# Bendabir/torch-kafka

Hardware: AMD Instinct MI355X
Metric: Kafka records/sec to GPU with per-batch commit, at 1/2/4/8 MI355X (higher is better)
Workload: dtype bf16

## Files before the change

torchkafka_amd/csrc/hip/json_span.hip:

```cpp
#include <hip/hip_runtime.h>

#include <stdexcept>
#include <string>

#include "dtypes.h"
#include "json_scan_dev.h"
#include "span_decode.h"
#include "span_device.h"

namespace tkh {

namespace {

using span::kBlock;
using span::kFront;
using span::kThreads;
using span::kWinBytes;
constexpr int kBufs = 2;
constexpr int kWaves = kThreads / 64;
constexpr int kMaxRows = int(tk::kJsonSpanMaxSegRows);
constexpr int kRowsPerThread = kMaxRows / kThreads;

__device__ __forceinline__ uint32_t align16(uint32_t x) { return (x + 15u) & ~15u; }

__global__ __launch_bounds__(kBlock) void json_stage_kernel(JsonStageLaunch a) {
  __shared__ __attribute__((aligned(16))) uint8_t bufs[kBufs][kWinBytes];
  __shared__ int32_t rel[kMaxRows];
  __shared__ int32_t tln[kMaxRows];
  __shared__ uint32_t dst[kMaxRows];
  __shared__ __attribute__((aligned(256))) uint32_t tab[span::kNibLdsWords];
  __shared__ span::RowWins rw;
  __shared__ uint32_t wcrc[kWaves];
  __shared__ uint32_t wsum[kWaves];
  __shared__ int32_t bad;

  const int t = int(threadIdx.x), lane = t & 63, wv = t >> 6;
  const int P = a.parts;
  const SpanDevSeg& sg = a.s[int(blockIdx.x) / P];
  const JsonStageBatch& bo = a.b[sg.batch];
  const uint32_t row_begin = sg.row_begin;
  const int32_t nrows = int32_t(sg.row_end - row_begin);
  const uint32_t flags = sg.flags;
  const int32_t trunc = bo.trunc_len;

  if (flags & tk::kSegHostRows) {
    if (wv != 0 || int(blockIdx.x) % P != 0) return;
    uint32_t off = sg.stage_off;
    for (int32_t rr = 0; rr < nrows; ++rr) {
      const int64_t row = int64_t(row_begin) + rr;
      const tk::JsonSpanRow d = bo.rows[row];
      if (d.tlen >= 0) continue;
      const int32_t n_out = trunc >= 0 && d.count > trunc ? trunc : d.count;
      const float* __restrict__ src = reinterpret_cast<const float*>(bo.slot + d.pos);
      float* __restrict__ o = reinterpret_cast<float*>(bo.stage + off);
      for (int32_t k = lane; k < n_out; k += 64) o[k] = src[k];
      if (lane == 0) {
        bo.desc[row] = JsonRowDesc{off, -1, d.count, n_out};
        if (bo.ctr) atomicMax(bo.ctr, (static_cast<unsigned long long>(bo.ctr_tag) << 32) | uint32_t(max(n_out, 0)));
      }
      off += align16(uint32_t(n_out) * 4u);
    }
    return;
  }

  const uint32_t len = sg.len;
  const int32_t head = int32_t(reinterpret_cast<uintptr_t>(sg.src) & 15u);
  const bool do_crc = (flags & tk::kSegCrc) != 0;
  const int32_t lo_b = kFront + head, hi_b = lo_b + int32_t(len);
  const span::Windows W(lo_b, hi_b);
  const span::Part pt = span::part_of(P, W.nw);

  const uint32_t crc = span::pipeline<kBufs>(
      sg.src, W, pt.k0, pt.k1, bufs, tab, a.tabs, lo_b + ((flags & tk::kSegCrcFirst) ? 21 : 0), do_crc,
      (flags & tk::kSegCrcFirst) != 0,
      [&] {
        const int64_t base = int64_t(sg.log_pos) - int64_t(head) - kFront;
        for (int32_t r = t; r < nrows; r += kThreads) {
          const tk::JsonSpanRow d = bo.rows[row_begin + uint32_t(r)];
          const int32_t r0 = d.tlen >= 0 ? int32_t(int64_t(d.pos) - base) : 0;
          rel[r] = r0;
          tln[r] = d.tlen < 0 ? -1 : (r0 < lo_b || r0 + d.tlen > hi_b) ? -2 : d.tlen;
        }
        span::row_wins_init(rw, W.nw);
        if (t == 0) bad = 0;
      },
      [&] {
        const bool cw = t < kThreads;
        uint32_t sz[kRowsPerThread], local = 0;
#pragma unroll
        for (int i = 0; i < kRowsPerThread; ++i) {
          const int32_t r = t * kRowsPerThread + i;
          sz[i] = cw && r < nrows && tln[r] >= 0 ? align16(uint32_t(tln[r])) : 0u;
          local += sz[i];
        }
        uint32_t incl = local;
#pragma unroll
        for (int o = 1; o < 64; o <<= 1) {
          const uint32_t u = __shfl_up(incl, o, 64);
          if (lane >= o) incl += u;
        }
        if (cw && lane == 63) wsum[wv] = incl;
        __syncthreads();
        if (!cw) return;
        uint32_t off = sg.stage_off + incl - local;
        for (int w = 0; w < wv; ++w) off += wsum[w];
#pragma unroll
        for (int i = 0; i < kRowsPerThread; ++i) {
          const int32_t r = t * kRowsPerThread + i;
          if (r < nrows) {
            dst[r] = off;
            const int32_t T = tln[r];
            if (pt.q != 0) {
            } else if (T == -2) {
              bo.desc[row_begin + uint32_t(r)] = JsonRowDesc{off, 0, 0, 0};
              bad = 1;
            } else if (T >= 0) {
              const int32_t c = bo.rows[row_begin + uint32_t(r)].count;
              const int32_t n_out = c < 0 ? 0 : trunc >= 0 && c > trunc ? trunc : c;
              bo.desc[row_begin + uint32_t(r)] = JsonRowDesc{off, T, c, n_out};
            }
          }
          off += sz[i];
        }
        for (int32_t r0w = 0; r0w < nrows; r0w += kThreads) {
          const int32_t r = r0w + t;
          const int32_t T = r < nrows ? tln[r] : -1;
          const int32_t r0 = r < nrows ? rel[r] : 0;
          span::row_wins_add(rw, W.nw, r0w + (t & ~63), T > 0, W.win_of(r0), W.win_of(r0 + ((T - 1) & ~15)));
        }
      },
      [&](int k, const uint8_t* buf, int32_t off) {
        const int32_t ra = rw.lo[k], rb = rw.hi[k];
        if (ra >= rb) return;
        const int32_t own_lo = W.own_lo(k), own_hi = W.own_hi(k);
        span::for_rows(
            ra, rb, false,
            [&](int32_t rr, int32_t* ulo, int32_t* uhi) {
              const int32_t T = tln[rr], r0 = rel[rr];
              *ulo = span::unit_from(r0, own_lo);
              *uhi = min(T > 0 ? (T + 15) >> 4 : 0, span::unit_from(r0, own_hi));
            },
            [&](int32_t rr, int32_t u) {
              *reinterpret_cast<uint4*>(bo.stage + dst[rr] + 16u * uint32_t(u)) =
                  span::lds16_row(reinterpret_cast<const uint4*>(buf), rel[rr] + 16 * u + off);
            });
      });

  if (do_crc) {
    if (t < kThreads) span::crc_merge(crc, wcrc);
    __syncthreads();
    if (t == 0)
      span::crc_finish(wcrc, flags, sg.crc, sg.seg, bo.err, bo.partials, P, pt.q,
                       a.part_acc + 2 * pt.seg);
  }
  if (t == 0 && bad) span::report_bad_segment(bo.err, sg.seg);
}

__global__ __launch_bounds__(256) void json_count_kernel(JsonGroupArgs a) {
  const int lane = int(threadIdx.x) & 63;
  const int64_t g = int64_t(blockIdx.x) * 4 + int64_t(threadIdx.x >> 6);
  if (g >= a.row_base[a.n]) return;
  int bk = 0;
#pragma unroll
  for (int k = 1; k < kMaxGroup; ++k) bk += (k < a.n && g >= a.row_base[k]) ? 1 : 0;
  if (!a.ctr[bk]) return;
  const int64_t r = g - a.row_base[bk];
  JsonRowDesc* desc = const_cast<JsonRowDesc*>(a.rows[bk]) + r;
  const JsonRowDesc d = *desc;
  if (d.count != tk::kJsonCountOnDevice || d.tlen < 0) return;
  const int32_t T = d.tlen;
  if (uint64_t(d.off) + ((uint64_t(T) + 15u) & ~uint64_t(15)) > a.vals_cap[bk]) return;
  const uint8_t* __restrict__ text = a.vals[bk] + d.off;
  int32_t guess = 0;
  const int32_t count = json_scan_row([&](int32_t c) { return *reinterpret_cast<const uint4*>(text + c); },
                                      [&](int32_t i) { return uint32_t(text[i]); }, T, lane, &guess);
  if (lane == 0) {
    const bool host = count < 0;
    const int32_t c = host ? guess : count;
    const int32_t trunc = a.trunc[bk];
    const int32_t n_out = trunc >= 0 && c > trunc ? trunc : c;
    *desc = JsonRowDesc{d.off, host ? tk::kJsonCountOnDevice : T, c, n_out};
    const unsigned long long tag = static_cast<unsigned long long>(a.ctr_tag[bk]) << 32;
    atomicMax(const_cast<unsigned long long*>(a.ctr[bk]), tag | uint32_t(max(n_out, 0)));
    if (host) atomicMax(const_cast<unsigned long long*>(a.ctr[bk]) + 1, tag | 1u);
  }
}

}

void launch_json_count(const JsonGroupArgs& a, hipStream_t stream) {
  if (a.n < 1 || a.n > kMaxGroup) throw std::invalid_argument("json count: group size out of range");
  const int64_t total = a.row_base[a.n];
  if (total <= 0) return;
  if (total > INT32_MAX) throw std::invalid_argument("json count: too many rows");
  for (int k = 0; k < a.n; ++k) {
    if (a.ctr[k] && (reinterpret_cast<uintptr_t>(a.vals[k]) % 16 || reinterpret_cast<uintptr_t>(a.rows[k]) % 16 ||
                     a.row_base[k + 1] < a.row_base[k]))
      throw std::invalid_argument("json count: malformed group");
  }
  hipLaunchKernelGGL(json_count_kernel, dim3(unsigned((total + 3) / 4)), dim3(256), 0, stream, a);
  hipError_t e = hipGetLastError();
  if (e != hipSuccess) throw std::runtime_error(std::string("json count launch: ") + hipGetErrorString(e));
}

void launch_json_stage(const JsonStageLaunch& a0, hipStream_t stream) {
  JsonStageLaunch a = a0;
  a.parts = check_parts(a.parts, a.part_acc, "json stage");
  if (a.n_seg < 0 || a.n_seg > kMaxLaunchSegs) throw std::invalid_argument("json stage: bad segment count");
  if (a.n_seg == 0) return;
  for (int i = 0; i < a.n_seg; ++i) {
    const SpanDevSeg& s = a.s[i];
    const bool host = (s.flags & tk::kSegHostRows) != 0;
    if ((!host && (s.len == 0 || s.len > tk::kSpanSegMax || s.src == nullptr)) || s.row_end < s.row_begin ||
        s.row_end - s.row_begin > tk::kJsonSpanMaxSegRows || s.batch >= kMaxGroup || a.b[s.batch].stage == nullptr ||
        a.b[s.batch].desc == nullptr || (s.stage_off & 15u) != 0)
      throw std::invalid_argument("json stage: malformed segment");
  }
  hipLaunchKernelGGL(json_stage_kernel, dim3(unsigned(a.n_seg * a.parts)), dim3(kBlock), 0, stream, a);
  hipError_t e = hipGetLastError();
  if (e != hipSuccess) throw std::runtime_error(std::string("json stage launch: ") + hipGetErrorString(e));
}

void prewarm_json_span_kernels() {
  hipFuncAttributes attr;
  (void)hipFuncGetAttributes(&attr, reinterpret_cast<const void*>(&json_stage_kernel));
  (void)hipFuncGetAttributes(&attr, reinterpret_cast<const void*>(&json_count_kernel));
}

}
```

torchkafka_amd/csrc/hip/span_decode.hip:

```cpp
#include <hip/hip_runtime.h>

#include <algorithm>
#include <stdexcept>
#include <string>

#include "convert.h"
#include "span_decode.h"
#include "span_device.h"

namespace tkh {

namespace {

using span::kBlock;
using span::kFront;
using span::kThreads;
using span::kWinBytes;
constexpr int kBufs = 3;

template <typename S>
__device__ __forceinline__ S lds_elem(const uint32_t* b32, int32_t b) {
  const int32_t w = b >> 2, sh = b & 3;
  if constexpr (sizeof(S) <= 4) {
    const uint32_t x = __builtin_amdgcn_alignbyte(b32[w + 1], b32[w], sh);
    S v;
    __builtin_memcpy(&v, &x, sizeof(S));
    return v;
  } else {
    const uint32_t x0 = b32[w], x1 = b32[w + 1], x2 = b32[w + 2];
    const uint32_t o[2] = {__builtin_amdgcn_alignbyte(x1, x0, sh), __builtin_amdgcn_alignbyte(x2, x1, sh)};
    S v;
    __builtin_memcpy(&v, o, sizeof(S));
    return v;
  }
}

template <typename S, typename D, bool AFFINE>
__global__ __launch_bounds__(kBlock) void span_decode_kernel(SpanLaunch a, const float* __restrict__ shift,
                                                               const float* __restrict__ scale) {
  using C = Conv<S, D, IsIntDst<D>::value>;
  constexpr int kPer = 16 / int(sizeof(S));
  __shared__ __attribute__((aligned(16))) uint8_t bufs[kBufs][kWinBytes];
  __shared__ int32_t rel[tk::kSpanMaxSegRows];
  __shared__ __attribute__((aligned(256))) uint32_t tab[span::kNibLdsWords];
  __shared__ span::RowWins rw;
  __shared__ uint32_t wcrc[kThreads / 64];

  const int t = int(threadIdx.x);
  const int P = a.parts;
  const SpanDevSeg& sg = a.s[int(blockIdx.x) / P];
  const SpanBatchOut& bo = a.b[sg.batch];
  const uint32_t len = sg.len, flags = sg.flags;
  const int32_t head = int32_t(reinterpret_cast<uintptr_t>(sg.src) & 15u);
  const uint32_t row_begin = sg.row_begin;
  const int32_t nrows = int32_t(sg.row_end - row_begin);
  const bool do_crc = (flags & tk::kSegCrc) != 0;
  const int32_t lo_b = kFront + head, hi_b = lo_b + int32_t(len);
  const span::Windows W(lo_b, hi_b);
  const span::Part pt = span::part_of(P, W.nw);
  const int64_t RE = a.row_elems;
  const int32_t G = int32_t((RE + kPer - 1) / kPer);
  const int32_t row_bytes = int32_t(RE * int64_t(sizeof(S)));
  D* __restrict__ out = static_cast<D*>(bo.out);

  auto group = [&](const uint8_t* buf, int32_t off, int32_t own_lo, int32_t own_hi, int32_t rr, int32_t gi,
                   bool row_wave) {
    const uint32_t* b32 = reinterpret_cast<const uint32_t*>(buf);
    const int32_t e0 = gi * kPer;
    const int32_t b0 = rel[rr] + e0 * int32_t(sizeof(S));
    const int64_t rem = RE - e0;
    const int nel = rem < kPer ? int(rem) : kPer;
    if (b0 + nel * int32_t(sizeof(S)) <= lo_b || b0 >= hi_b) return;
    const int32_t key = b0 > lo_b ? b0 : lo_b;
    if (key < own_lo || key >= own_hi) return;
    D* __restrict__ orow = out + int64_t(row_begin + uint32_t(rr)) * RE;
    if (nel == kPer && b0 >= lo_b && b0 + 16 <= hi_b) {
      const uint4 o = row_wave ? span::lds16_row(reinterpret_cast<const uint4*>(buf), b0 + off)
                               : span::lds16(reinterpret_cast<const uint4*>(buf), b0 + off);
      S sv[kPer];
      __builtin_memcpy(sv, &o, 16);
      Vec<D, kPer> ov;
#pragma unroll
      for (int k = 0; k < kPer; ++k) {
        if constexpr (AFFINE)
          ov.v[k] = C::apply(sv[k], shift[e0 + k], scale[e0 + k], true);
        else
          ov.v[k] = C::apply(sv[k], 0.f, 1.f, false);
      }
      if (a.vec_store) {
        *reinterpret_cast<Vec<D, kPer>*>(orow + e0) = ov;
      } else {
#pragma unroll
        for (int k = 0; k < kPer; ++k) orow[e0 + k] = ov.v[k];
      }
    } else {
      for (int k = 0; k < nel; ++k) {
        const int32_t be = b0 + k * int32_t(sizeof(S));
        if (be < lo_b || be + int32_t(sizeof(S)) > hi_b) continue;
        const S sv = lds_elem<S>(b32, be + off);
        if constexpr (AFFINE)
          orow[e0 + k] = C::apply(sv, shift[e0 + k], scale[e0 + k], true);
        else
          orow[e0 + k] = C::apply(sv, 0.f, 1.f, false);
      }
    }
  };

  const uint32_t crc = span::pipeline<kBufs>(
      sg.src, W, pt.k0, pt.k1, bufs, tab, a.tabs, lo_b + ((flags & tk::kSegCrcFirst) ? 21 : 0), do_crc,
      (flags & tk::kSegCrcFirst) != 0,
      [&] {
        const int64_t base = int64_t(sg.log_pos) - int64_t(head) - kFront;
        for (int32_t r = t; r < nrows; r += kThreads) rel[r] = int32_t(int64_t(bo.row_pos[row_begin + uint32_t(r)]) - base);
        span::row_wins_init(rw, W.nw);
      },
      [&] {
        if (t >= kThreads) return;
        for (int32_t r0w = 0; r0w < nrows; r0w += kThreads) {
          const int32_t r = r0w + t;
          const int32_t r0 = r < nrows ? rel[r] : 0;
          const bool in = r < nrows && r0 + row_bytes > lo_b && r0 < hi_b;
          const int32_t kf = r0 > lo_b ? r0 : lo_b, kl = min(r0 + (G - 1) * 16, hi_b - 1);
          span::row_wins_add(rw, W.nw, r0w + (t & ~63), in, W.win_of(kf), W.win_of(kl));
        }
        if (sg.seg == 0 && pt.q == 0 && bo.ext_words)
          for (uint32_t i = uint32_t(t); i < bo.ext_words; i += kThreads) bo.ext_out[i] = bo.ext_src[i];
      },
      [&](int k, const uint8_t* buf, int32_t off) {
        const int32_t ra = rw.lo[k], rb = rw.hi[k];
        if (ra >= rb) return;
        const int32_t own_lo = W.own_lo(k), own_hi = W.own_hi(k);
        if (G >= 32) {
          span::for_rows(
              ra, rb, G > 128,
              [&](int32_t rr, int32_t* ulo, int32_t* uhi) {
                const int32_t r0 = rel[rr];
                *ulo = k == 0 ? (r0 >= lo_b ? 0 : (lo_b - r0) >> 4) : span::unit_from(r0, own_lo);
                *uhi = min(G, span::unit_from(r0, own_hi));
              },
              [&](int32_t rr, int32_t gi) { group(buf, off, own_lo, own_hi, rr, gi, true); });
        } else {
          const int32_t total = (rb - ra) * G;
          for (int32_t p = t; p < total; p += kThreads) {
            const int32_t q = p / G;
            group(buf, off, own_lo, own_hi, ra + q, p - q * G, false);
          }
        }
      });

  if (do_crc) {
    if (t < kThreads) span::crc_merge(crc, wcrc);
    __syncthreads();
    if (t == 0)
      span::crc_finish(wcrc, flags, sg.crc, sg.seg, bo.err, bo.partials, P, pt.q,
                       a.part_acc + 2 * pt.seg);
  }
}

template <typename S, typename D>
__global__ __launch_bounds__(kBlock) void varlen_span_kernel(VarSpanLaunch a, D pad) {
  using C = Conv<S, D, IsIntDst<D>::value>;
  constexpr int kWaves = kThreads / 64;
  constexpr int kPer = 16 / int(sizeof(S));
  __shared__ __attribute__((aligned(16))) uint8_t bufs[kBufs][kWinBytes];
  __shared__ int32_t rel[tk::kJsonSpanMaxSegRows];
  __shared__ int32_t nout[tk::kJsonSpanMaxSegRows];
  __shared__ __attribute__((aligned(256))) uint32_t tab[span::kNibLdsWords];
  __shared__ span::RowWins rw;
  __shared__ uint32_t wcrc[kWaves];
  __shared__ int32_t bad;

  const int t = int(threadIdx.x), lane = t & 63, wv = t >> 6;
  const int P = a.parts;
  const SpanDevSeg& sg = a.s[int(blockIdx.x) / P];
  const VarSpanBatch& bo = a.b[sg.batch];
  const uint32_t row_begin = sg.row_begin;
  const int32_t nrows = int32_t(sg.row_end - row_begin);
  const uint32_t flags = sg.flags;
  const int64_t L = bo.L;
  const int32_t trunc = bo.trunc_len;
  D* __restrict__ out = static_cast<D*>(bo.out);
  auto finish = [&](D* orow, int64_t row, int64_t n_out) {
    for (int64_t k = n_out + lane; k < L; k += 64) orow[k] = pad;
    if (bo.mask) {
      uint8_t* mrow = bo.mask + row * L;
      for (int64_t k = lane; k < L; k += 64) mrow[k] = uint8_t(k < n_out);
    }
    if (bo.lengths && lane == 0) bo.lengths[row] = n_out;
  };

  if (flags & tk::kSegHostRows) {
    if (wv >= kWaves || int(blockIdx.x) % P != 0) return;
    for (int32_t rr = wv; rr < nrows; rr += kWaves) {
      const int64_t row = int64_t(row_begin) + rr;
      const tk::JsonSpanRow d = bo.rows[row];
      if (d.tlen >= 0) continue;
      int64_t n_out = trunc >= 0 && d.count > trunc ? trunc : d.count;
      n_out = n_out < L ? n_out : L;
      const S* __restrict__ v = reinterpret_cast<const S*>(bo.slot + d.pos);
      D* orow = out + row * L;
      for (int64_t k = lane; k < n_out; k += 64) orow[k] = C::apply(v[k], 0.f, 1.f, false);
      finish(orow, row, n_out);
    }
    return;
  }

  const uint32_t len = sg.len;
  const int32_t head = int32_t(reinterpret_cast<uintptr_t>(sg.src) & 15u);
  const bool do_crc = (flags & tk::kSegCrc) != 0;
  const int32_t lo_b = kFront + head, hi_b = lo_b + int32_t(len);
  const span::Windows W(lo_b, hi_b);
  const span::Part pt = span::part_of(P, W.nw);

  const uint32_t crc = span::pipeline<kBufs>(
      sg.src, W, pt.k0, pt.k1, bufs, tab, a.tabs, lo_b + ((flags & tk::kSegCrcFirst) ? 21 : 0), do_crc,
      (flags & tk::kSegCrcFirst) != 0,
      [&] {
        const int64_t base = int64_t(sg.log_pos) - int64_t(head) - kFront;
        for (int32_t r = t; r < nrows; r += kThreads) {
          const tk::JsonSpanRow d = bo.rows[row_begin + uint32_t(r)];
          rel[r] = d.tlen >= 0 ? int32_t(int64_t(d.pos) - base) : 0;
          int32_t n = -1;
          if (d.tlen >= 0) {
            int64_t n_out = trunc >= 0 && d.count > trunc ? trunc : d.count;
            n_out = n_out < L ? n_out : L;
            const bool ok = rel[r] >= lo_b && rel[r] + d.tlen <= hi_b && int64_t(d.count) * int64_t(sizeof(S)) == d.tlen;
            n = ok ? int32_t(n_out) : -2;
          }
          nout[r] = n;
        }
        span::row_wins_init(rw, W.nw);
        if (t == 0) bad = 0;
      },
      [&] {
        if (t >= kThreads) return;
        for (int32_t rr = wv; rr < nrows; rr += kWaves) {
          const int32_t n = nout[rr];
          if (n == -1) continue;
          if (n == -2 && lane == 0) bad = 1;
          const int64_t row = int64_t(row_begin) + rr;
          if (pt.q == 0) finish(out + row * L, row, n < 0 ? 0 : n);
        }
        for (int32_t r0w = 0; r0w < nrows; r0w += kThreads) {
          const int32_t r = r0w + t;
          const int32_t n = r < nrows ? nout[r] : 0;
          const int32_t r0 = r < nrows ? rel[r] : 0;
          const int32_t units = n > 0 ? (n + kPer - 1) / kPer : 0;
          span::row_wins_add(rw, W.nw, r0w + (t & ~63), units > 0, W.win_of(r0), W.win_of(r0 + 16 * (units - 1)));
        }
      },
      [&](int k, const uint8_t* buf, int32_t off) {
        const int32_t ra = rw.lo[k], rb = rw.hi[k];
        if (ra >= rb) return;
        const int32_t own_lo = W.own_lo(k), own_hi = W.own_hi(k);
        const uint32_t* b32 = reinterpret_cast<const uint32_t*>(buf);
        span::for_rows(
            ra, rb, false,
            [&](int32_t rr, int32_t* ulo, int32_t* uhi) {
              const int32_t n = nout[rr], r0 = rel[rr];
              const int32_t units = n > 0 ? (n + kPer - 1) / kPer : 0;
              *ulo = span::unit_from(r0, own_lo);
              *uhi = min(units, span::unit_from(r0, own_hi));
            },
            [&](int32_t rr, int32_t u) {
              const int32_t n = nout[rr], r0 = rel[rr];
              D* orow = out + (int64_t(row_begin) + rr) * L;
              const int32_t e0 = u * kPer, b0 = r0 + 16 * u + off;
              if (bo.reserved && e0 + kPer <= n) {
                const uint4 o = span::lds16_row(reinterpret_cast<const uint4*>(buf), b0);
                S sv[kPer];
                __builtin_memcpy(sv, &o, 16);
                Vec<D, kPer> ov;
#pragma unroll
                for (int q = 0; q < kPer; ++q) ov.v[q] = C::apply(sv[q], 0.f, 1.f, false);
                *reinterpret_cast<Vec<D, kPer>*>(orow + e0) = ov;
              } else {
                for (int q = 0; q < kPer && e0 + q < n; ++q)
                  orow[e0 + q] = C::apply(lds_elem<S>(b32, b0 + q * int32_t(sizeof(S))), 0.f, 1.f, false);
              }
            });
      });

  if (do_crc) {
    if (t < kThreads) span::crc_merge(crc, wcrc);
    __syncthreads();
    if (t == 0)
      span::crc_finish(wcrc, flags, sg.crc, sg.seg, bo.err, bo.partials, P, pt.q,
                       a.part_acc + 2 * pt.seg);
  }
  if (t == 0 && bad) span::report_bad_segment(bo.err, sg.seg);
}

template <typename S, typename D>
void launch_var_span_t(const VarSpanLaunch& a, double pad, hipStream_t stream) {
  D padv;
  if constexpr (IsIntDst<D>::value) padv = D(int64_t(pad)); else padv = Store<D>::cvt(float(pad));
  hipLaunchKernelGGL((varlen_span_kernel<S, D>), dim3(unsigned(a.n_seg * a.parts)), dim3(kBlock), 0, stream, a, padv);
}

template <typename S, typename D>
void launch_span_t(const SpanLaunch& a, const float* shift, const float* scale, hipStream_t stream) {
  if (a.n_seg <= 0) return;
  const dim3 grid(unsigned(a.n_seg * a.parts));
  if (shift)
    hipLaunchKernelGGL((span_decode_kernel<S, D, true>), grid, dim3(kBlock), 0, stream, a, shift, scale);
  else
    hipLaunchKernelGGL((span_decode_kernel<S, D, false>), grid, dim3(kBlock), 0, stream, a, shift, scale);
}

}

int check_parts(int parts, const uint32_t* acc, const char* what) {
  if (parts <= 1) return 1;
  if ((parts != 2 && parts != 4 && parts != tk::kSpanMaxParts) || acc == nullptr)
    throw std::invalid_argument(std::string(what) + ": parts must be 1, 2, 4 or 8 (with accumulator words)");
  return parts;
}

void prewarm_span_kernels(int device) {
  (void)device;
  hipFuncAttributes attr;
  (void)hipFuncGetAttributes(&attr, reinterpret_cast<const void*>(&span_decode_kernel<float, __bf16, false>));
  (void)hipFuncGetAttributes(&attr, reinterpret_cast<const void*>(&span_decode_kernel<float, float, false>));
  (void)hipFuncGetAttributes(&attr, reinterpret_cast<const void*>(&span_decode_kernel<float, _Float16, false>));
  (void)hipFuncGetAttributes(&attr, reinterpret_cast<const void*>(&span_decode_kernel<float, fp8e4m3, false>));
}

void check_var_span(const VarSpanLaunch& a, int src_dt, int dst_dt) {
  check_parts(a.parts, a.part_acc, "var span");
  if (a.n_seg < 0 || a.n_seg > kMaxLaunchSegs) throw std::invalid_argument("var span: bad segment count");
  if (!is_float_dt(dst_dt) && is_float_dt(src_dt))
    throw std::invalid_argument("collate: float records cannot be cast to an integer dtype");
  for (int i = 0; i < a.n_seg; ++i) {
    const SpanDevSeg& s = a.s[i];
    const bool host = (s.flags & tk::kSegHostRows) != 0;
    if ((!host && (s.len == 0 || s.len > tk::kSpanSegMax || s.src == nullptr)) || s.row_end < s.row_begin ||
        s.row_end - s.row_begin > tk::kJsonSpanMaxSegRows || s.batch >= kMaxGroup ||
        (a.b[s.batch].L > 0 && a.b[s.batch].out == nullptr))
      throw std::invalid_argument("var span: malformed segment");
    const VarSpanBatch& b = a.b[s.batch];
    if (b.err == nullptr || (s.row_end > s.row_begin && (b.rows == nullptr || (host && b.slot == nullptr))) ||
        (!host && (s.flags & tk::kSegCrc) && (a.tabs == nullptr || b.partials == nullptr)))
      throw std::invalid_argument("var span: a segment without its status word, row table, slot or CRC tables");
  }
}

void launch_var_span(const VarSpanLaunch& a0, int src_dt, int dst_dt, double pad, hipStream_t stream) {
  check_var_span(a0, src_dt, dst_dt);
  VarSpanLaunch a = a0;
  a.parts = check_parts(a.parts, a.part_acc, "var span");
  if (a.n_seg == 0) return;
  TK_DISPATCH_SRC(launch_var_span_t, a, pad, stream)
  hipError_t e = hipGetLastError();
  if (e != hipSuccess) throw std::runtime_error(std::string("var span launch: ") + hipGetErrorString(e));
}

void check_span_decode(const SpanLaunch& a, int src_dt, int dst_dt, const float* shift, const float* scale) {
  check_parts(a.parts, a.part_acc, "span decode");
  if (a.n_seg < 0 || a.n_seg > kMaxLaunchSegs) throw std::invalid_argument("span decode: bad segment count");
  if (!is_float_dt(dst_dt) && is_float_dt(src_dt))
    throw std::invalid_argument("collate: float records cannot be cast to an integer dtype");
  if (shift && !is_float_dt(dst_dt)) throw std::invalid_argument("collate: normalisation needs a float dtype");
  if ((shift == nullptr) != (scale == nullptr)) throw std::invalid_argument("span decode: shift and scale go together");
  if (a.n_seg > 0 && a.row_elems < 1) throw std::invalid_argument("span decode: row_elems must be positive");
  for (int i = 0; i < a.n_seg; ++i) {
    const SpanDevSeg& s = a.s[i];
    if (s.len == 0 || s.len > tk::kSpanSegMax || s.src == nullptr || s.row_end < s.row_begin ||
        s.row_end - s.row_begin > tk::kSpanMaxSegRows || s.batch >= kMaxGroup)
      throw std::invalid_argument("span decode: malformed segment");
    const SpanBatchOut& b = a.b[s.batch];
    if ((s.row_end > s.row_begin && (b.out == nullptr || b.row_pos == nullptr)) ||
        ((s.flags & tk::kSegCrc) && (a.tabs == nullptr || b.err == nullptr || b.partials == nullptr)) ||
        (b.ext_words && (b.ext_out == nullptr || b.ext_src == nullptr)))
      throw std::invalid_argument("span decode: a segment without its output, row table, status words or CRC tables");
  }
}

void launch_span_decode(const SpanLaunch& a0, int src_dt, int dst_dt, const float* shift, const float* scale,
                        hipStream_t stream) {
  check_span_decode(a0, src_dt, dst_dt, shift, scale);
  SpanLaunch a = a0;
  a.parts = check_parts(a.parts, a.part_acc, "span decode");
  TK_DISPATCH_SRC(launch_span_t, a, shift, scale, stream)
  hipError_t e = hipGetLastError();
  if (e != hipSuccess) throw std::runtime_error(std::string("span decode launch: ") + hipGetErrorString(e));
}

}
```

torchkafka_amd/csrc/hip/span_device.h:

```cpp
#pragma once
#include <hip/hip_runtime.h>

#include <cstdint>

#include "span.h"

namespace tkh {
namespace span {

constexpr int kThreads = int(tk::kSpanLanes);
constexpr int kBlock = kThreads + 64;
constexpr int kFront = 16;
constexpr int32_t kWin = int32_t(tk::kSpanWin);
constexpr int kPad = tk::kSpanWinPad;
constexpr int kWinBytes = tk::kSpanWinBytes;
constexpr int kWinLoads = tk::kSpanWinLoads;
static_assert(kWinBytes % 16 == 0, "window buffers stay 16-byte aligned");
static_assert(kWinLoads <= 21, "counted waits: at most 3 windows of loads in flight (vmcnt <= 63)");
static_assert(kThreads == 512, "crc_merge / crc_finish: 8 compute waves, one lane constant per thread");

__device__ __forceinline__ bool loader_wave() { return threadIdx.x >= kThreads; }

typedef uint32_t lds_v4u __attribute__((ext_vector_type(4)));
__device__ __forceinline__ uint4 lds16(const uint4* img16, int32_t b0) {
  const lds_v4u* img = reinterpret_cast<const lds_v4u*>(img16);
  const int32_t q = (b0 >> 2) & 3, sh = b0 & 3;
  const lds_v4u lv = __builtin_nontemporal_load(img + (b0 >> 4));
  const lds_v4u hv = __builtin_nontemporal_load(img + (b0 >> 4) + 1);
  const uint4 lo = make_uint4(lv.x, lv.y, lv.z, lv.w), hi = make_uint4(hv.x, hv.y, hv.z, hv.w);
  const uint32_t d0 = q == 0 ? lo.x : q == 1 ? lo.y : q == 2 ? lo.z : lo.w;
  const uint32_t d1 = q == 0 ? lo.y : q == 1 ? lo.z : q == 2 ? lo.w : hi.x;
  const uint32_t d2 = q == 0 ? lo.z : q == 1 ? lo.w : q == 2 ? hi.x : hi.y;
  const uint32_t d3 = q == 0 ? lo.w : q == 1 ? hi.x : q == 2 ? hi.y : hi.z;
  const uint32_t d4 = q == 0 ? hi.x : q == 1 ? hi.y : q == 2 ? hi.z : hi.w;
  uint4 v;
  v.x = __builtin_amdgcn_alignbyte(d1, d0, sh);
  v.y = __builtin_amdgcn_alignbyte(d2, d1, sh);
  v.z = __builtin_amdgcn_alignbyte(d3, d2, sh);
  v.w = __builtin_amdgcn_alignbyte(d4, d3, sh);
  return v;
}

__device__ __forceinline__ uint4 lds16_row(const uint4* img16, int32_t b0) {
  const lds_v4u* img = reinterpret_cast<const lds_v4u*>(img16);
  const int32_t a = __builtin_amdgcn_readfirstlane(b0 & 15), q = a >> 2, sh = a & 3;
  const lds_v4u lv = __builtin_nontemporal_load(img + (b0 >> 4));
  const lds_v4u hv = __builtin_nontemporal_load(img + (b0 >> 4) + 1);
  uint32_t d[5];
  if (q == 0) {
    d[0] = lv.x, d[1] = lv.y, d[2] = lv.z, d[3] = lv.w, d[4] = hv.x;
  } else if (q == 1) {
    d[0] = lv.y, d[1] = lv.z, d[2] = lv.w, d[3] = hv.x, d[4] = hv.y;
  } else if (q == 2) {
    d[0] = lv.z, d[1] = lv.w, d[2] = hv.x, d[3] = hv.y, d[4] = hv.z;
  } else {
    d[0] = lv.w, d[1] = hv.x, d[2] = hv.y, d[3] = hv.z, d[4] = hv.w;
  }
  uint4 v;
  v.x = __builtin_amdgcn_alignbyte(d[1], d[0], sh);
  v.y = __builtin_amdgcn_alignbyte(d[2], d[1], sh);
  v.z = __builtin_amdgcn_alignbyte(d[3], d[2], sh);
  v.w = __builtin_amdgcn_alignbyte(d[4], d[3], sh);
  return v;
}

__device__ __forceinline__ uint32_t keep_from(int32_t a, int32_t c) {
  const int32_t d = c - a;
  return d <= 0 ? 0xFFFFFFFFu : d >= 4 ? 0u : (0xFFFFFFFFu << (8 * d));
}

__device__ __forceinline__ uint32_t gf_mul(uint32_t k, uint32_t c) {
  uint32_t p = 0;
#pragma unroll
  for (int i = 31; i >= 0; --i) {
    p ^= c & uint32_t(int32_t(k << (31 - i)) >> 31);
    c = (c >> 1) ^ (0x82F63B78u & uint32_t(int32_t(c << 31) >> 31));
  }
  return p;
}

using Windows = tk::SpanWindows;

__device__ __forceinline__ void issue_window(const uint8_t* gbase, const Windows& W, int k, uint8_t* buf) {
  const int lane = int(threadIdx.x) & 63;
  const int32_t a = W.stage_lo(k);
  const int32_t last = ((W.stage_hi(k) - a) >> 4) - 1;
  const uint8_t* g = gbase + (a - kFront);
#pragma unroll
  for (int r = 0; r < kWinLoads; ++r) {
    const int32_t c = min(r * 64 + lane, last);
    __builtin_amdgcn_global_load_lds(g + 16 * c, (__attribute__((address_space(3))) void*)(buf + kPad + 1024 * r), 16,
                                     0, 0);
  }
}

__device__ __forceinline__ void loader_wait(int n) {
  if (n <= 0)
    asm volatile("s_waitcnt vmcnt(0)" ::: "memory");
  else if (n == 1)
    asm volatile("s_waitcnt vmcnt(%0)" ::"n"(kWinLoads) : "memory");
  else
    asm volatile("s_waitcnt vmcnt(%0)" ::"n"(2 * kWinLoads) : "memory");
}

__device__ __forceinline__ void window_barrier() {
  asm volatile("s_waitcnt lgkmcnt(0)" ::: "memory");
  __builtin_amdgcn_s_barrier();
  asm volatile("" ::: "memory");
}

struct RowWins {
  int32_t lo[32], hi[32];
};
__device__ __forceinline__ void row_wins_init(RowWins& rw, int nw) {
  const int t = int(threadIdx.x);
  if (t < nw) {
    rw.lo[t] = 0x7FFFFFFF;
    rw.hi[t] = 0;
  }
}
__device__ __forceinline__ void row_wins_add(RowWins& rw, int nw, int32_t row_base, bool valid, int kf, int kl) {
  const int lane = int(threadIdx.x) & 63;
  for (int k = 0; k < nw; ++k) {
    const unsigned long long m = __ballot(valid && kf <= k && k <= kl);
    if (m && lane == 0) {
      atomicMin(&rw.lo[k], row_base + int32_t(__builtin_ctzll(m)));
      atomicMax(&rw.hi[k], row_base + 64 - int32_t(__builtin_clzll(m)));
    }
  }
}

template <class Range, class Fn>
__device__ __forceinline__ void for_rows(int32_t ra, int32_t rb, bool wide, Range&& range, Fn&& fn) {
  const int t = int(threadIdx.x), lane = t & 63, wv = t >> 6;
  const int32_t r_step = wide ? 1 : kThreads / 64, c_off = wide ? 64 * wv : 0, c_step = wide ? kThreads : 64;
  for (int32_t rr = ra + (wide ? 0 : wv); rr < rb; rr += r_step) {
    int32_t ulo = 0, uhi = 0;
    range(rr, &ulo, &uhi);
    for (int32_t u = ulo + c_off + lane; u < uhi; u += c_step) fn(rr, u);
  }
}
__device__ __forceinline__ int32_t unit_from(int32_t key0, int32_t x) { return key0 >= x ? 0 : (x - key0 + 15) >> 4; }

constexpr int kNibRowWords = 64;
constexpr int kNibLdsWords = 16 * kNibRowWords;
using lds_u32 = __attribute__((address_space(3))) const uint32_t;

__device__ __forceinline__ void load_nib_rows(uint32_t* tab, const uint32_t* __restrict__ tabs) {
  for (int i = int(threadIdx.x); i < int(tk::kSpanTabNibWords); i += kThreads)
    tab[(i >> 4) * kNibRowWords + (i & 15)] = tabs[tk::kSpanTabNib + i];
  for (int i = int(threadIdx.x); i < int(tk::kSpanTabGapWords); i += kThreads)
    tab[(i >> 4) * kNibRowWords + 16 + (i & 15)] = tabs[tk::kSpanTabGap + i];
}

template <int B>
__device__ __forceinline__ uint32_t nib_dword(uint32_t nbase, uint32_t w) {
  const uint32_t lo = (w << 2) & 0x3C3C3C3Cu, hi = (w >> 2) & 0x3C3C3C3Cu;
  uint32_t r = 0;
#pragma unroll
  for (int i = 0; i < 4; ++i) {
    const uint32_t sel = 0x07060500u | uint32_t(i);
    const uint32_t a0 = __builtin_amdgcn_perm(nbase + uint32_t(2 * (B - i)) * 256u, lo, sel);
    const uint32_t a1 = __builtin_amdgcn_perm(nbase + uint32_t(2 * (B - i) + 1) * 256u, hi, sel);
    r ^= *(lds_u32*)uintptr_t(a0) ^ *(lds_u32*)uintptr_t(a1);
  }
  return r;
}

__device__ __forceinline__ uint32_t gap_op(uint32_t nbase, uint32_t c) {
  uint32_t r = 0;
#pragma unroll
  for (int i = 0; i < 8; ++i) r ^= *(lds_u32*)uintptr_t(nbase + uint32_t(i) * 256u + 64u + ((c >> (4 * i)) & 15u) * 4u);
  return r;
}

__device__ __forceinline__ uint32_t crc_piece(const uint32_t* __restrict__ b32, uint32_t nbase, const Windows& W,
                                              int k, int32_t off, int32_t c0, bool first, uint32_t crc) {
  const int t = int(threadIdx.x);
  constexpr int32_t P = int32_t(tk::kSpanPiece);
  constexpr int32_t nsteps = (P - 4) >> 3;
  if (k > 0) crc = gap_op(nbase, crc);
  const int32_t start = W.w0 + k * kWin + t * P + off;
  const int32_t cl = c0 + off;
  const int32_t sh = start & 3;
  int32_t w = start >> 2;
  if (start >= cl + 4) {
    uint32_t lo = b32[w + 1];
    crc = nib_dword<3>(nbase, __builtin_amdgcn_alignbyte(lo, b32[w], sh) ^ crc);
#pragma unroll
    for (int32_t j = 0; j < nsteps; ++j) {
      const uint32_t m1 = b32[w + 2 + 2 * j], m2 = b32[w + 3 + 2 * j];
      const uint32_t x = __builtin_amdgcn_alignbyte(m1, lo, sh) ^ crc, y = __builtin_amdgcn_alignbyte(m2, m1, sh);
      lo = m2;
      crc = nib_dword<7>(nbase, x) ^ nib_dword<3>(nbase, y);
    }
    return crc;
  }
  if (start + 4 > cl) {
    uint32_t x = __builtin_amdgcn_alignbyte(b32[w + 1], b32[w], sh);
    const uint32_t keep = keep_from(start, cl);
    x &= keep;
    if (first) x ^= keep & ~keep_from(start, cl + 4);
    crc = nib_dword<3>(nbase, x ^ crc);
  }
  const int32_t a1 = start + 4;
  const int32_t j0 = a1 >= cl ? 0 : (cl - a1) >> 3;
  if (j0 < nsteps) {
    int32_t ad = a1 + 8 * j0;
    w = ad >> 2;
    uint32_t lo = b32[w];
    for (int32_t j = j0; j < nsteps; ++j, ad += 8) {
      const uint32_t m1 = b32[w + 1], m2 = b32[w + 2];
      w += 2;
      uint32_t x = __builtin_amdgcn_alignbyte(m1, lo, sh), y = __builtin_amdgcn_alignbyte(m2, m1, sh);
      lo = m2;
      if (ad < cl + 4) {
        const uint32_t kx = keep_from(ad, cl), ky = keep_from(ad + 4, cl);
        x &= kx;
        y &= ky;
        if (first) {
          x ^= kx & ~keep_from(ad, cl + 4);
          y ^= ky & ~keep_from(ad + 4, cl + 4);
        }
      }
      x ^= crc;
      crc = nib_dword<7>(nbase, x) ^ nib_dword<3>(nbase, y);
    }
  }
  return crc;
}

__device__ __forceinline__ void crc_merge(uint32_t crc, uint32_t* wcrc) {
  const int t = int(threadIdx.x), lane = t & 63;
#pragma unroll
  for (int j = 32; j >= 1; j >>= 1) crc ^= uint32_t(__shfl_xor(int(crc), j, 64));
  if (lane == 0) wcrc[t >> 6] = crc;
}

struct Part {
  int32_t seg, q, k0, k1;
};
__device__ __forceinline__ Part part_of(int parts, int32_t nw) {
  const int32_t b = int32_t(blockIdx.x), seg = b / parts, q = b - seg * parts;
  return Part{seg, q, tk::span_part_k0(q, parts, nw), tk::span_part_k0(q + 1, parts, nw)};
}

__device__ __forceinline__ void report_bad_segment(int32_t* err, uint32_t seg) {
  uint32_t* w = reinterpret_cast<uint32_t*>(err);
  uint32_t cur = __hip_atomic_load(w, __ATOMIC_RELAXED, __HIP_MEMORY_SCOPE_SYSTEM);
  while (seg < cur && !__hip_atomic_compare_exchange_strong(w, &cur, seg, __ATOMIC_RELAXED, __ATOMIC_RELAXED,
                                                            __HIP_MEMORY_SCOPE_SYSTEM)) {
  }
  if (int32_t(__hip_atomic_load(w, __ATOMIC_RELAXED, __HIP_MEMORY_SCOPE_SYSTEM)) < 0) *err = int32_t(seg);
}

__device__ __forceinline__ void crc_finish(const uint32_t* wcrc, uint32_t flags, uint32_t want, uint32_t seg,
                                           int32_t* err, uint32_t* partials, int parts, int q, uint32_t* acc) {
  uint32_t c = 0;
#pragma unroll
  for (int i = 0; i < kThreads / 64; ++i) c ^= wcrc[i];
  if (parts > 1) {
    auto* word = reinterpret_cast<unsigned long long*>(acc);
    const uint32_t bit = 1u << q;
    const unsigned long long old = __hip_atomic_fetch_xor(word, (static_cast<unsigned long long>(bit) << 32) | c,
                                                          __ATOMIC_RELAXED, __HIP_MEMORY_SCOPE_AGENT);
    if ((uint32_t(old >> 32) | bit) != (1u << parts) - 1u) return;
    c ^= uint32_t(old);
    __hip_atomic_exchange(word, 0ull, __ATOMIC_RELAXED, __HIP_MEMORY_SCOPE_AGENT);
  }
  constexpr uint32_t kWhole = tk::kSegCrcFirst | tk::kSegCrcLast;
  if ((flags & kWhole) == kWhole) {
    if ((c ^ 0xFFFFFFFFu) != want) report_bad_segment(err, seg);
  } else {
    partials[seg] = c;
  }
}

template <int NB, class Setup, class Prepare, class Body>
__device__ __forceinline__ uint32_t pipeline(const uint8_t* src, const Windows& W, int32_t k0, int32_t k1,
                                             uint8_t (*bufs)[kWinBytes], uint32_t* tab,
                                             const uint32_t* __restrict__ tabs, int32_t c0, bool do_crc, bool first,
                                             Setup&& setup, Prepare&& prepare, Body&& body) {
  static_assert(NB >= 2 && NB <= 4, "2..4 window buffers");
  const uint8_t* gbase = reinterpret_cast<const uint8_t*>(reinterpret_cast<uintptr_t>(src) & ~uintptr_t(15));
  const bool loader = loader_wave();
  if (loader) {
    for (int j = 0; j < NB - 1 && k0 + j < k1; ++j) issue_window(gbase, W, k0 + j, bufs[j]);
  } else {
    if (do_crc) load_nib_rows(tab, tabs);
    setup();
  }
  window_barrier();
  prepare();
  __syncthreads();
  const uint32_t nbase = uint32_t(uintptr_t((lds_u32*)tab));
  const uint32_t lane_k =
      do_crc && !loader ? tabs[tk::kSpanTabLaneMul + uint32_t(W.nw - k1) * tk::kSpanLanes + threadIdx.x] : 0u;
  uint32_t crc = 0;
  for (int k = k0; k < k1; ++k) {
    const int j = k - k0;
    if (loader) {
      loader_wait(min(k + NB - 2, k1 - 1) - k);
      window_barrier();
      if (k + NB - 1 < k1) issue_window(gbase, W, k + NB - 1, bufs[(j + NB - 1) % NB]);
    } else {
      window_barrier();
      uint8_t* buf = bufs[j % NB];
      const int32_t off = kPad - W.stage_lo(k);
#ifndef TKH_SPAN_PROBE_NO_BODY
      body(k, buf, off);
#endif
#ifndef TKH_SPAN_PROBE_NO_CRC
      if (do_crc) crc = crc_piece(reinterpret_cast<const uint32_t*>(buf), nbase, W, k, off, c0, first, crc);
#endif
    }
  }
  return do_crc && !loader ? gf_mul(lane_k, crc) : 0u;
}

}
}
```

Measured before the change: 45.04 million.

## Hoist per-row and CRC table global loads ahead of the first pipeline barrier

The span-decode pipeline now gets a fetch callback. Compute waves issue their first row descriptor and CRC table words (nib, gap and lane multiplier) up front, before an initial barrier, so the global-load latency overlaps with the loader wave starting its window loads. The loader and compute paths are split into separate loops. __syncthreads is replaced by a raw s_barrier wrapper, and the ring depth can now be set with a macro while counted waits are generalised per ring size. The risks are subtle synchronisation mistakes, since the barrier counts must match between the loader and compute paths, and extra register pressure from the held values.

Result: no change. 44.84 million (-0.4%).

```diff
diff --git a/torchkafka_amd/csrc/hip/json_span.hip b/torchkafka_amd/csrc/hip/json_span.hip
--- a/torchkafka_amd/csrc/hip/json_span.hip
+++ b/torchkafka_amd/csrc/hip/json_span.hip
@@ -73,10 +73,11 @@
   const uint32_t crc = span::pipeline<kBufs>(
       sg.src, W, pt.k0, pt.k1, bufs, tab, a.tabs, lo_b + ((flags & tk::kSegCrcFirst) ? 21 : 0), do_crc,
       (flags & tk::kSegCrcFirst) != 0,
-      [&] {
+      [&] { return t < nrows ? bo.rows[row_begin + uint32_t(t)] : tk::JsonSpanRow{0, 0, 0}; },
+      [&](const tk::JsonSpanRow& row_t) {
         const int64_t base = int64_t(sg.log_pos) - int64_t(head) - kFront;
         for (int32_t r = t; r < nrows; r += kThreads) {
-          const tk::JsonSpanRow d = bo.rows[row_begin + uint32_t(r)];
+          const tk::JsonSpanRow d = r == t ? row_t : bo.rows[row_begin + uint32_t(r)];
           const int32_t r0 = d.tlen >= 0 ? int32_t(int64_t(d.pos) - base) : 0;
           rel[r] = r0;
           tln[r] = d.tlen < 0 ? -1 : (r0 < lo_b || r0 + d.tlen > hi_b) ? -2 : d.tlen;
@@ -100,7 +101,7 @@
           if (lane >= o) incl += u;
         }
         if (cw && lane == 63) wsum[wv] = incl;
-        __syncthreads();
+        span::lds_barrier();
         if (!cw) return;
         uint32_t off = sg.stage_off + incl - local;
         for (int w = 0; w < wv; ++w) off += wsum[w];
@@ -148,7 +149,7 @@
 
   if (do_crc) {
     if (t < kThreads) span::crc_merge(crc, wcrc);
-    __syncthreads();
+    span::lds_barrier();
     if (t == 0)
       span::crc_finish(wcrc, flags, sg.crc, sg.seg, bo.err, bo.partials, P, pt.q,
                        a.part_acc + 2 * pt.seg);
diff --git a/torchkafka_amd/csrc/hip/span_decode.hip b/torchkafka_amd/csrc/hip/span_decode.hip
--- a/torchkafka_amd/csrc/hip/span_decode.hip
+++ b/torchkafka_amd/csrc/hip/span_decode.hip
@@ -16,7 +16,10 @@
 using span::kFront;
 using span::kThreads;
 using span::kWinBytes;
-constexpr int kBufs = 3;
+#ifndef TKH_SPAN_RING
+#define TKH_SPAN_RING 3
+#endif
+constexpr int kBufs = TKH_SPAN_RING;
 
 template <typename S>
 __device__ __forceinline__ S lds_elem(const uint32_t* b32, int32_t b) {
@@ -109,9 +112,12 @@
   const uint32_t crc = span::pipeline<kBufs>(
       sg.src, W, pt.k0, pt.k1, bufs, tab, a.tabs, lo_b + ((flags & tk::kSegCrcFirst) ? 21 : 0), do_crc,
       (flags & tk::kSegCrcFirst) != 0,
-      [&] {
+      [&] { return t < nrows ? bo.row_pos[row_begin + uint32_t(t)] : uint64_t(0); },
+      [&](uint64_t pos_t) {
         const int64_t base = int64_t(sg.log_pos) - int64_t(head) - kFront;
-        for (int32_t r = t; r < nrows; r += kThreads) rel[r] = int32_t(int64_t(bo.row_pos[row_begin + uint32_t(r)]) - base);
+        if (t < nrows) rel[t] = int32_t(int64_t(pos_t) - base);
+        for (int32_t r = t + kThreads; r < nrows; r += kThreads)
+          rel[r] = int32_t(int64_t(bo.row_pos[row_begin + uint32_t(r)]) - base);
         span::row_wins_init(rw, W.nw);
       },
       [&] {
@@ -150,7 +156,7 @@
 
   if (do_crc) {
     if (t < kThreads) span::crc_merge(crc, wcrc);
-    __syncthreads();
+    span::lds_barrier();
     if (t == 0)
       span::crc_finish(wcrc, flags, sg.crc, sg.seg, bo.err, bo.partials, P, pt.q,
                        a.part_acc + 2 * pt.seg);
@@ -215,10 +221,11 @@
   const uint32_t crc = span::pipeline<kBufs>(
       sg.src, W, pt.k0, pt.k1, bufs, tab, a.tabs, lo_b + ((flags & tk::kSegCrcFirst) ? 21 : 0), do_crc,
       (flags & tk::kSegCrcFirst) != 0,
-      [&] {
+      [&] { return t < nrows ? bo.rows[row_begin + uint32_t(t)] : tk::JsonSpanRow{0, 0, 0}; },
+      [&](const tk::JsonSpanRow& row_t) {
         const int64_t base = int64_t(sg.log_pos) - int64_t(head) - kFront;
         for (int32_t r = t; r < nrows; r += kThreads) {
-          const tk::JsonSpanRow d = bo.rows[row_begin + uint32_t(r)];
+          const tk::JsonSpanRow d = r == t ? row_t : bo.rows[row_begin + uint32_t(r)];
           rel[r] = d.tlen >= 0 ? int32_t(int64_t(d.pos) - base) : 0;
           int32_t n = -1;
           if (d.tlen >= 0) {
@@ -283,7 +290,7 @@
 
   if (do_crc) {
     if (t < kThreads) span::crc_merge(crc, wcrc);
-    __syncthreads();
+    span::lds_barrier();
     if (t == 0)
       span::crc_finish(wcrc, flags, sg.crc, sg.seg, bo.err, bo.partials, P, pt.q,
                        a.part_acc + 2 * pt.seg);
diff --git a/torchkafka_amd/csrc/hip/span_device.h b/torchkafka_amd/csrc/hip/span_device.h
--- a/torchkafka_amd/csrc/hip/span_device.h
+++ b/torchkafka_amd/csrc/hip/span_device.h
@@ -16,7 +16,6 @@
 constexpr int kWinBytes = tk::kSpanWinBytes;
 constexpr int kWinLoads = tk::kSpanWinLoads;
 static_assert(kWinBytes % 16 == 0, "window buffers stay 16-byte aligned");
-static_assert(kWinLoads <= 21, "counted waits: at most 3 windows of loads in flight (vmcnt <= 63)");
 static_assert(kThreads == 512, "crc_merge / crc_finish: 8 compute waves, one lane constant per thread");
 
 __device__ __forceinline__ bool loader_wave() { return threadIdx.x >= kThreads; }
@@ -94,13 +93,18 @@
   }
 }
 
+template <int NB>
 __device__ __forceinline__ void loader_wait(int n) {
+  static_assert(NB >= 2 && NB <= 4 && (NB - 1) * kWinLoads <= 63, "counted waits: the vmcnt field holds 63");
+  static_assert(NB * kWinLoads <= 63, "a full ring of loads in flight stays within the counter");
   if (n <= 0)
     asm volatile("s_waitcnt vmcnt(0)" ::: "memory");
-  else if (n == 1)
+  else if (n == 1 || NB == 2)
     asm volatile("s_waitcnt vmcnt(%0)" ::"n"(kWinLoads) : "memory");
+  else if (n == 2 || NB == 3)
+    asm volatile("s_waitcnt vmcnt(%0)" ::"n"(2 * kWinLoads) : "memory");
   else
-    asm volatile("s_waitcnt vmcnt(%0)" ::"n"(2 * kWinLoads) : "memory");
+    asm volatile("s_waitcnt vmcnt(%0)" ::"n"(3 * kWinLoads) : "memory");
 }
 
 __device__ __forceinline__ void window_barrier() {
@@ -108,6 +112,7 @@
   __builtin_amdgcn_s_barrier();
   asm volatile("" ::: "memory");
 }
+__device__ __forceinline__ void lds_barrier() { window_barrier(); }
 
 struct RowWins {
   int32_t lo[32], hi[32];
@@ -146,11 +151,23 @@
 constexpr int kNibLdsWords = 16 * kNibRowWords;
 using lds_u32 = __attribute__((address_space(3))) const uint32_t;
 
-__device__ __forceinline__ void load_nib_rows(uint32_t* tab, const uint32_t* __restrict__ tabs) {
-  for (int i = int(threadIdx.x); i < int(tk::kSpanTabNibWords); i += kThreads)
-    tab[(i >> 4) * kNibRowWords + (i & 15)] = tabs[tk::kSpanTabNib + i];
-  for (int i = int(threadIdx.x); i < int(tk::kSpanTabGapWords); i += kThreads)
-    tab[(i >> 4) * kNibRowWords + 16 + (i & 15)] = tabs[tk::kSpanTabGap + i];
+struct CrcWords {
+  uint32_t nib, gap, lane_k;
+};
+static_assert(tk::kSpanTabNibWords <= uint32_t(kThreads) && tk::kSpanTabGapWords <= uint32_t(kThreads),
+              "one table word per compute thread");
+__device__ __forceinline__ CrcWords fetch_crc_words(const uint32_t* __restrict__ tabs, uint32_t after) {
+  const uint32_t i = threadIdx.x;
+  CrcWords c;
+  c.nib = i < tk::kSpanTabNibWords ? tabs[tk::kSpanTabNib + i] : 0u;
+  c.gap = i < tk::kSpanTabGapWords ? tabs[tk::kSpanTabGap + i] : 0u;
+  c.lane_k = tabs[tk::kSpanTabLaneMul + after * tk::kSpanLanes + i];
+  return c;
+}
+__device__ __forceinline__ void store_nib_rows(uint32_t* tab, const CrcWords& c) {
+  const int i = int(threadIdx.x);
+  if (i < int(tk::kSpanTabNibWords)) tab[(i >> 4) * kNibRowWords + (i & 15)] = c.nib;
+  if (i < int(tk::kSpanTabGapWords)) tab[(i >> 4) * kNibRowWords + 16 + (i & 15)] = c.gap;
 }
 
 template <int B>
@@ -276,47 +293,58 @@
   }
 }
 
-template <int NB, class Setup, class Prepare, class Body>
+template <int NB, class Fetch, class Setup, class Prepare, class Body>
 __device__ __forceinline__ uint32_t pipeline(const uint8_t* src, const Windows& W, int32_t k0, int32_t k1,
                                              uint8_t (*bufs)[kWinBytes], uint32_t* tab,
                                              const uint32_t* __restrict__ tabs, int32_t c0, bool do_crc, bool first,
-                                             Setup&& setup, Prepare&& prepare, Body&& body) {
+                                             Fetch&& fetch, Setup&& setup, Prepare&& prepare, Body&& body) {
   static_assert(NB >= 2 && NB <= 4, "2..4 window buffers");
   const uint8_t* gbase = reinterpret_cast<const uint8_t*>(reinterpret_cast<uintptr_t>(src) & ~uintptr_t(15));
   const bool loader = loader_wave();
+  const int n = k1 - k0;
+  CrcWords cw{0u, 0u, 0u};
+  decltype(fetch()) f{};
+  if (!loader) {
+    if (do_crc) cw = fetch_crc_words(tabs, uint32_t(W.nw - k1));
+    f = fetch();
+  }
+  asm volatile("" ::: "memory");
+  __builtin_amdgcn_s_barrier();
+  asm volatile("" ::: "memory");
   if (loader) {
-    for (int j = 0; j < NB - 1 && k0 + j < k1; ++j) issue_window(gbase, W, k0 + j, bufs[j]);
-  } else {
-    if (do_crc) load_nib_rows(tab, tabs);
-    setup();
-  }
+    __builtin_amdgcn_s_waitcnt(0x0F70);
+    for (int j = 0; j < NB - 1 && j < n; ++j) issue_window(gbase, W, k0 + j, bufs[j]);
+    window_barrier();
+    prepare();
+    window_barrier();
+    for (int j = 0; j < n; ++j) {
+      loader_wait<NB>(min(j + NB - 1, n) - 1 - j);
+      window_barrier();
+      if (j + NB - 1 < n) issue_window(gbase, W, k0 + j + NB - 1, bufs[(j + NB - 1) % NB]);
+    }
+    return 0u;
+  }
+  if (do_crc) store_nib_rows(tab, cw);
+  setup(f);
   window_barrier();
   prepare();
-  __syncthreads();
+  window_barrier();
   const uint32_t nbase = uint32_t(uintptr_t((lds_u32*)tab));
-  const uint32_t lane_k =
-      do_crc && !loader ? tabs[tk::kSpanTabLaneMul + uint32_t(W.nw - k1) * tk::kSpanLanes + threadIdx.x] : 0u;
   uint32_t crc = 0;
-  for (int k = k0; k < k1; ++k) {
-    const int j = k - k0;
-    if (loader) {
-      loader_wait(min(k + NB - 2, k1 - 1) - k);
-      window_barrier();
-      if (k + NB - 1 < k1) issue_window(gbase, W, k + NB - 1, bufs[(j + NB - 1) % NB]);
-    } else {
-      window_barrier();
-      uint8_t* buf = bufs[j % NB];
-      const int32_t off = kPad - W.stage_lo(k);
+  for (int j = 0; j < n; ++j) {
+    const int k = k0 + j;
+    window_barrier();
+    uint8_t* buf = bufs[j % NB];
+    const int32_t off = kPad - W.stage_lo(k);
 #ifndef TKH_SPAN_PROBE_NO_BODY
-      body(k, buf, off);
+    body(k, buf, off);
 #endif
 #ifndef TKH_SPAN_PROBE_NO_CRC
-      if (do_crc) crc = crc_piece(reinterpret_cast<const uint32_t*>(buf), nbase, W, k, off, c0, first, crc);
+    if (do_crc) crc = crc_piece(reinterpret_cast<const uint32_t*>(buf), nbase, W, k, off, c0, first, crc);
 #endif
-    }
-  }
-  return do_crc && !loader ? gf_mul(lane_k, crc) : 0u;
-}
-
-}
-}
+  }
+  return do_crc ? gf_mul(cw.lane_k, crc) : 0u;
+}
+
+}
+}
```
